# jurgisp/pydreamer

Measured on AMD Instinct MI355X. Metric: grad-steps/sec (world-model+AC) at B=50,T=50,H=15, 64×64 obs, 1/2/4/8 GPU, higher is better.
Workload: dtype f32; 1 GPU; atari-literal: defaults+atari, batch_size 50, batch_length 50, imag_horizon 15, deter_dim 600, stoch 32x32, hidden 1000, cnn_depth 48, action_dim 18, fp32; fwd + 4 bwd + clip + 4 AdamW per step; replay resident in HBM; global_batch=50, batch_length=50, imag_horizon=15, parallelism=dp1 (batch-sharded [50])

## Files before the change

### include/dreamer_hip.h

```cpp
#ifndef DREAMER_HIP_H
#define DREAMER_HIP_H

#include <stddef.h>
#include <stdint.h>

#ifdef __cplusplus
extern "C" {
#endif

#define DM_OK 0
#define DM_E_SHAPE (-1)
#define DM_E_WORKSPACE (-2)
#define DM_E_HIP (-3)
#define DM_E_DEVICE (-4)
#define DM_E_NULL (-5)

#define DM_MAX_MLP_LAYERS 8

typedef struct dm_shape {
  int32_t T, B, I;
  int32_t H;
  int32_t D, Hd;
  int32_t S, C;
  int32_t E;
  int32_t A;
  int32_t mlp_hidden;
  int32_t mlp_layers;
  int32_t cnn_depth;
  int32_t img, img_ch;
  int32_t flags;
} dm_shape;
#define DM_FLAG_IMAGE_U8 16
#define DM_FLAG_GRU_SHIFT 5
#define DM_FLAG_BF16 128
#define DM_FLAG_GRU_LAYERS_SHIFT 8
#define DM_FLAG_GRU_LAYERS_MASK (3 << DM_FLAG_GRU_LAYERS_SHIFT)
#define DM_FLAG_GRU_MASK (3 << DM_FLAG_GRU_SHIFT)

int dm_version(void);
const char* dm_last_error(void);
int dm_device_check(void);
size_t dm_workspace_bytes(const dm_shape* shp);
int dm_stream_create_cu_mask(const uint32_t* mask, int words, void** stream);
int dm_stream_destroy(void* stream);
int dm_wgrad_side_arm(int on);
int dm_wgrad_side_touch(void);
int dm_wgrad_side_join(void* stream);

#define DM_GEMM_ACCUM 1
#define DM_GEMM_ELU 2
#define DM_GEMM_BF16 256
int dm_gemm_f32(int a_layout, int b_layout, int M, int N, int K,
                const float* A, int lda, const float* B, int ldb, float* C, int ldc,
                const float* bias, const float* add, int ldadd, int flags,
                void* ws, size_t ws_bytes, void* stream);
int dm_gemm_bf16h(int a_layout, int b_layout, int M, int N, int K, const uint16_t* A, int lda, const uint16_t* B, int ldb,
                  float* C, int ldc, uint16_t* C_h, const float* bias, int flags, void* ws, size_t ws_bytes, void* stream);
int dm_bf16_twins_enable(int on);
int dm_gemm_dma_enable(int on);
int dm_convt_kskip_enable(int on);
int dm_kl_staged_enable(int on);
int dm_dec_l4_bwd_direct_enable(int on);
int dm_dec_l4_fwd_shared_enable(int on);
int dm_rssm_lds_enable(int on);
int dm_bptt_fold_enable(int on);
int dm_rssm_lds_status(void);
int dm_rssm_lds_status_ack(void);
int dm_rssm_lds_gave_up(void);
int dm_rssm_lds_prof(unsigned long long* out16, int reset);

int dm_ln_elu_fwd(int rows, int n, const float* x, int ldx, const float* gamma, const float* beta, float eps,
                  float* y, int ldy, float* stats, void* stream);
int dm_ln_elu_bwd(int rows, int n, const float* x, int ldx, const float* y, int ldy, const float* stats,
                  const float* gamma, const float* dy, int lddy, float* dx, int lddx,
                  float* dgamma, float* dbeta, void* ws, size_t ws_bytes, void* stream);
int dm_colsum(int rows, int n, const float* x, int ld, float* out, void* ws, size_t ws_bytes, void* stream);

int dm_gru_gates_fwd(int rows, int D, const float* gi, const float* gh, const float* h_in, int ldh,
                     float* h_out, int ldo, void* stream);
int dm_gru_gates_bwd(int rows, int D, const float* gi, const float* gh, const float* h_in, int ldh,
                     const float* dh_out, int lddh, float* dgi, float* dgh, float* dh_in, int lddi, void* stream);

int dm_sample_onehot(int rows, int groups, int C, const float* logits, int ldl, const float* u,
                     const int32_t* forced_idx, float* onehot, int ldo, int32_t* idx, void* stream);

int dm_kl_balance_fwd(int rows, int S, int C, const float* post, const float* prior,
                      float* kl, float* ent_post, float* ent_prior, void* stream);
int dm_kl_balance_bwd(int rows, int S, int C, const float* post, const float* prior,
                      float scale_post, float scale_prior, float* dpost, float* dprior, void* stream);
int dm_st_softmax_bwd(int rows, int groups, int C, const float* logits, int ldl, const float* dz, int lddz,
                      float* dlogits, int lddl, int accum, void* stream);

int dm_kl_sampled_fwd(int rows, int S, int C, const float* post, const float* prior, const int32_t* idx, float* out, void* stream);
int dm_kl_sampled_bwd(int rows, int S, int C, const float* post, const float* prior, const int32_t* idx, float scale,
                      const float* row_w, float* dpost, float* dprior, void* stream);
int dm_kl_sampled_gauss_fwd(int rows, int S, const float* post, const float* prior, const float* z, int ldz, float* out,
                            void* stream);
int dm_kl_sampled_gauss_bwd(int rows, int S, const float* post, const float* prior, const float* z, int ldz, float scale,
                            const float* row_w, float* dpost, float* dprior, float* dz, int lddz, void* stream);
int dm_reduce_i(int TB, int I, int W, const float* x, int mode, float* out, float* w_out, void* stream);
int dm_combine_rows(int count, int64_t n, const float* const* x, const float* w, float* out, void* stream);
int dm_scale_rows(int64_t rows, int n, float* x, int ldx, const float* w, float scale, void* stream);

int dm_mask_rows(int rows, int n, const float* x, int ldx, const uint8_t* reset, float* y, int ldy, void* stream);

int dm_im2col_s2(int n, int hb, int wb, int c, int k, const float* big, int big_nchw, float* col, void* stream);
#define DM_C2I_ELU 1
int dm_col2im_s2(int n, int hb, int wb, int c, int k, const float* col, const float* bias, int flags,
                 const float* elu_ref, float* big, void* stream);

typedef struct dm_mlp_params {
  const float* w[DM_MAX_MLP_LAYERS + 1];
  const float* b[DM_MAX_MLP_LAYERS + 1];
  const float* ln_g[DM_MAX_MLP_LAYERS];
  const float* ln_b[DM_MAX_MLP_LAYERS];
  int32_t precision;
  int32_t reserved_;
} dm_mlp_params;
typedef struct dm_mlp_grads {
  float* w[DM_MAX_MLP_LAYERS + 1];
  float* b[DM_MAX_MLP_LAYERS + 1];
  float* ln_g[DM_MAX_MLP_LAYERS];
  float* ln_b[DM_MAX_MLP_LAYERS];
} dm_mlp_grads;
size_t dm_mlp_acts_floats(int rows, int hidden, int layers);
size_t dm_mlp_ws_floats(int rows, int hidden, int layers);
int dm_mlp_head_fwd(int rows, int in_dim, int hidden, int layers, int out_dim,
                    const float* x, int ldx, const dm_mlp_params* p, float* acts, float* out,
                    void* ws, size_t ws_bytes, void* stream);
int dm_mlp_head_fwd_sparse(int rows, int in_dim, int sparse_cols, int hidden, int layers, int out_dim,
                           const float* x, int ldx, const dm_mlp_params* p, float* acts, float* out,
                           void* ws, size_t ws_bytes, void* stream);
int dm_mlp_head_fwd_rows(int rows_total, int row0, int rows, int in_dim, int sparse_cols, int hidden, int layers, int out_dim,
                         const float* x, int ldx, const dm_mlp_params* p, float* acts, float* out,
                         void* ws, size_t ws_bytes, void* stream);

int dm_mlp_head_bwd(int rows, int in_dim, int hidden, int layers, int out_dim,
                    const float* x, int ldx, const dm_mlp_params* p, const float* acts, const float* dout,
                    const dm_mlp_grads* g, float* dx, int lddx, int dx_accum,
                    void* ws, size_t ws_bytes, void* stream);

int dm_head_loss(int kind, int rows, const float* out, const float* target, float scale, float loss_const,
                 float* loss, float* dout, float* mean_out, void* stream);

int dm_head_loss_normal_nd(int rows, int V, const float* out, const float* target, float scale, float loss_const,
                           float* loss, float* dout, float* mean_out, void* stream);
// ... 163 lines not shown
```

### pydreamer_amd/csrc/conv_direct.hip

```cpp
#include "common.h"

static inline int grid_for_px(size_t total, int per_block) { return (int)((total + per_block - 1) / per_block); }


template <int CO, bool U8, bool FB = false>
__global__ void __launch_bounds__(256) enc_l1_fwd_kernel(int npix, const void* __restrict__ image_,
                                                         const float* __restrict__ wt, const float* __restrict__ bias,
                                                         float* __restrict__ y, unsigned short* __restrict__ y_h) {
  const int p = blockIdx.x * 256 + threadIdx.x;
  const bool ok = p < npix;
  const int pc = ok ? p : npix - 1;
  const int n = pc / 961, r = pc - n * 961, py = r / 31, px = r - py * 31;
  float acc[CO];
  if (FB) {
    const float4* fb = reinterpret_cast<const float4*>(bias + (size_t)n * CO);
#pragma unroll
    for (int o = 0; o < CO; o += 4) {
      const float4 b4 = fb[o >> 2];
      acc[o] = b4.x; acc[o + 1] = b4.y; acc[o + 2] = b4.z; acc[o + 3] = b4.w;
    }
  } else {
#pragma unroll
    for (int o = 0; o < CO; ++o) acc[o] = bias[o];
  }
#pragma unroll 1
  for (int cy = 0; cy < 12; ++cy) {
    const int c = cy >> 2, ky = cy & 3;
    float v[4];
    if (U8) {
      const uint8_t* img = (const uint8_t*)image_ + (size_t)n * 12288 + ((size_t)(2 * py + ky) * 64 + 2 * px) * 3 + c;
#pragma unroll
      for (int kx = 0; kx < 4; ++kx) v[kx] = (float)img[kx * 3] / 255.0f - 0.5f;
    } else {
      const float* img = (const float*)image_ + (size_t)n * 12288 + (size_t)c * 4096 + (2 * py + ky) * 64 + 2 * px;
      const float2 a = *reinterpret_cast<const float2*>(img), b = *reinterpret_cast<const float2*>(img + 2);
      v[0] = a.x; v[1] = a.y; v[2] = b.x; v[3] = b.y;
    }
    const float* w = wt + (size_t)(c * 16 + ky * 4) * CO;
#pragma unroll
    for (int kx = 0; kx < 4; ++kx)
#pragma unroll
      for (int o = 0; o < CO; ++o) acc[o] = fmaf(v[kx], w[kx * CO + o], acc[o]);
  }
  if (ok) {
    float4* dst = reinterpret_cast<float4*>(y + (size_t)p * CO);
#pragma unroll
    for (int o = 0; o < CO; o += 4)
      dst[o >> 2] = make_float4(dm_elu(acc[o]), dm_elu(acc[o + 1]), dm_elu(acc[o + 2]), dm_elu(acc[o + 3]));
    if (y_h) {
      uint2* dh = reinterpret_cast<uint2*>(y_h + (size_t)p * CO);
#pragma unroll
      for (int o = 0; o < CO; o += 4)
        dh[o >> 2] = dm_pack_bf16x4(make_float4(dm_elu(acc[o]), dm_elu(acc[o + 1]), dm_elu(acc[o + 2]), dm_elu(acc[o + 3])));
    }
  }
}

template <int WROW = 48>
__global__ void __launch_bounds__(256) enc_l1_wt_kernel(int co, const float* __restrict__ w, float* __restrict__ wt) {
  const int e = blockIdx.x * 256 + threadIdx.x;
  if (e < co * 48) wt[e] = w[(size_t)(e % co) * WROW + e / co];
}
__global__ void __launch_bounds__(256) enc_l1_fb_kernel(int frames, int co, const float* __restrict__ w5,
                                                        const float* __restrict__ bias, const float* __restrict__ reward,
                                                        const float* __restrict__ terminal, float* __restrict__ fb) {
  const int e = blockIdx.x * 256 + threadIdx.x;
  if (e >= frames * co) return;
  const int n = e / co, o = e - n * co;
  const float* w = w5 + (size_t)o * 80 + 48;
  float s3 = 0.f, s4 = 0.f;
#pragma unroll
  for (int t = 0; t < 16; ++t) { s3 += w[t]; s4 += w[16 + t]; }
  fb[e] = fmaf(terminal[n], s4, fmaf(reward[n], s3, bias[o]));
}

bool dm_enc_l1_direct_ok(int ch, int d, int img) {
  return ch == 3 && img == 64 && (d == 8 || d == 16 || d == 32 || d == 48 || d == 64);
}
int dm_enc_l1_fwd_launch(int frames, int d, int u8, const void* image, const float* w, const float* bias, float* wt,
                         float* y, unsigned short* y_h, hipStream_t st) {
  if (frames <= 0) return DM_OK;
  hipLaunchKernelGGL(enc_l1_wt_kernel<48>, dim3(grid_for_px((size_t)d * 48, 256)), dim3(256), 0, st, d, w, wt);
  DM_LAUNCH_CHECK();
  const int npix = frames * 961;
  const dim3 grid(grid_for_px((size_t)npix, 256)), blk(256);
#define DM_ENC_L1(CO_)                                                                                              \
  if (d == CO_) {                                                                                                   \
    if (u8) hipLaunchKernelGGL((enc_l1_fwd_kernel<CO_, true>), grid, blk, 0, st, npix, image, wt, bias, y, y_h);      \
    else hipLaunchKernelGGL((enc_l1_fwd_kernel<CO_, false>), grid, blk, 0, st, npix, image, wt, bias, y, y_h);        \
  }
  DM_ENC_L1(8) DM_ENC_L1(16) DM_ENC_L1(32) DM_ENC_L1(48) DM_ENC_L1(64)
#undef DM_ENC_L1
  DM_LAUNCH_CHECK();
  return DM_OK;
}

int dm_enc_l1_fwd_planes_launch(int frames, int d, int u8, const void* image, const float* w5, const float* bias,
                                const float* reward, const float* terminal, float* wt, float* fb, float* y,
                                unsigned short* y_h, hipStream_t st) {
  if (frames <= 0) return DM_OK;
  hipLaunchKernelGGL(enc_l1_wt_kernel<80>, dim3(grid_for_px((size_t)d * 48, 256)), dim3(256), 0, st, d, w5, wt);
  DM_LAUNCH_CHECK();
  hipLaunchKernelGGL(enc_l1_fb_kernel, dim3(grid_for_px((size_t)frames * d, 256)), dim3(256), 0, st, frames, d, w5, bias, reward,
                     terminal, fb);
  DM_LAUNCH_CHECK();
  const int npix = frames * 961;
  const dim3 grid(grid_for_px((size_t)npix, 256)), blk(256);
#define DM_ENC_L1P(CO_)                                                                                             \
  if (d == CO_) {                                                                                                   \
    if (u8) hipLaunchKernelGGL((enc_l1_fwd_kernel<CO_, true, true>), grid, blk, 0, st, npix, image, wt, fb, y, y_h);  \
    else hipLaunchKernelGGL((enc_l1_fwd_kernel<CO_, false, true>), grid, blk, 0, st, npix, image, wt, fb, y, y_h);    \
  }
  DM_ENC_L1P(8) DM_ENC_L1P(16) DM_ENC_L1P(32) DM_ENC_L1P(48) DM_ENC_L1P(64)
#undef DM_ENC_L1P
  DM_LAUNCH_CHECK();
  return DM_OK;
}

typedef float f32x4c __attribute__((ext_vector_type(4)));
constexpr int ENC_LD = 68;
template <int OB, bool U8>
__global__ void __launch_bounds__(256) enc_l1_wgrad_kernel(int frames, int CO, const void* __restrict__ image_,
                                                           const float* __restrict__ G, float* __restrict__ part) {
  __shared__ __attribute__((aligned(16))) float img[3 * 64 * ENC_LD];
  const int tid = threadIdx.x, lane = tid & 63, wave = tid >> 6;
  const int l15 = lane & 15, q = lane >> 4;
  f32x4c acc[OB][3];
#pragma unroll
  for (int i = 0; i < OB; ++i)
#pragma unroll
    for (int j = 0; j < 3; ++j) acc[i][j] = (f32x4c){0.f, 0.f, 0.f, 0.f};
  const int tapoff = (l15 >> 2) * ENC_LD + (l15 & 3);
  for (int n = blockIdx.x; n < frames; n += gridDim.x) {
    __syncthreads();
    if (U8) {
      const uint8_t* src = (const uint8_t*)image_ + (size_t)n * 12288;
      for (int e = tid; e < 12288; e += 256) {
        const int c = e % 3, pix = e / 3;
        img[(c * 64 + (pix >> 6)) * ENC_LD + (pix & 63)] = (float)src[e] / 255.0f - 0.5f;
      }
    } else {
      const float4* src = reinterpret_cast<const float4*>((const float*)image_ + (size_t)n * 12288);
      for (int e = tid; e < 3072; e += 256) {
        const int row = e >> 4, c4 = e & 15;
        *reinterpret_cast<float4*>(&img[row * ENC_LD + 4 * c4]) = src[e];
      }
    }
    __syncthreads();
    const float* Gn = G + (size_t)n * 961 * CO;
    for (int p0 = wave * 64; p0 < 961; p0 += 256) {
      float a[16][OB];
#pragma unroll
      for (int ks = 0; ks < 16; ++ks) {
        const int p = p0 + 4 * ks + q;
        const int pc = p < 961 ? p : 960;
#pragma unroll
        for (int ob = 0; ob < OB; ++ob) {
          const int o = ob * 16 + l15;
          a[ks][ob] = Gn[(size_t)pc * CO + (o < CO ? o : CO - 1)] * ((p < 961 && o < CO) ? 1.f : 0.f);
        }
      }
#pragma unroll
      for (int ks = 0; ks < 16; ++ks) {
        const int p = p0 + 4 * ks + q;
        const int pc = p < 961 ? p : 960;
        const int py = pc / 31, px = pc - py * 31;
        const float* base = &img[2 * py * ENC_LD + 2 * px + tapoff];
        float b[3];
#pragma unroll
        for (int c = 0; c < 3; ++c) b[c] = base[c * 64 * ENC_LD];
#pragma unroll
        for (int ob = 0; ob < OB; ++ob)
#pragma unroll
          for (int c = 0; c < 3; ++c) acc[ob][c] = __builtin_amdgcn_mfma_f32_16x16x4f32(a[ks][ob], b[c], acc[ob][c], 0, 0, 0);
      }
    }
  }
  float* dst = part + (size_t)(blockIdx.x * 4 + wave) * CO * 48;
#pragma unroll
  for (int ob = 0; ob < OB; ++ob)
#pragma unroll
    for (int c = 0; c < 3; ++c)
#pragma unroll
      for (int r = 0; r < 4; ++r) {
        const int o = ob * 16 + 4 * q + r;
        if (o < CO) dst[(size_t)o * 48 + c * 16 + l15] = acc[ob][c][r];
      }
}

static int enc_l1_wgrad_blocks(int frames) { return frames > 512 ? 512 : frames; }
size_t dm_enc_l1_wgrad_part_floats(int frames, int d) { return (size_t)enc_l1_wgrad_blocks(frames) * 4 * d * 48; }
int dm_enc_l1_wgrad_launch(int frames, int d, int u8, const void* image, const float* G, float* part, float* dW, void* ws,
                           size_t ws_bytes, hipStream_t st) {
  if (frames <= 0) return DM_OK;
  const int blocks = enc_l1_wgrad_blocks(frames);
  const dim3 grid(blocks), blk(256);
  const int OB = (d + 15) / 16;
  DM_REQUIRE(OB >= 1 && OB <= 4, DM_E_SHAPE, "enc_l1_wgrad: cnn_depth %d", d);
#define DM_ENC_WG(OB_)                                                                                               \
  if (OB == OB_) {                                                                                                   \
    if (u8) hipLaunchKernelGGL((enc_l1_wgrad_kernel<OB_, true>), grid, blk, 0, st, frames, d, image, G, part);         \
    else hipLaunchKernelGGL((enc_l1_wgrad_kernel<OB_, false>), grid, blk, 0, st, frames, d, image, G, part);           \
  }
  DM_ENC_WG(1) DM_ENC_WG(2) DM_ENC_WG(3) DM_ENC_WG(4)
#undef DM_ENC_WG
  DM_LAUNCH_CHECK();
  return dm_colsum_launch(blocks * 4, d * 48, part, d * 48, dW, ws, ws_bytes, st);
}

__global__ void __launch_bounds__(256) enc_l1_planes_colsum_kernel(int frames, int d, int W, int frames_per_chunk,
                                                                   const float* __restrict__ G, const float* __restrict__ reward,
                                                                   const float* __restrict__ terminal, float* __restrict__ part) {
  __shared__ float sh[3][256];
  const int tid = threadIdx.x;
  const int n0 = blockIdx.x * frames_per_chunk, n1 = min(frames, n0 + frames_per_chunk);
  const int fl = 961 * d;
  float a0 = 0.f, a1 = 0.f, a2 = 0.f;
  if (tid < W)
    for (int n = n0; n < n1; ++n) {
      const float* x = G + (size_t)n * fl;
      float b0 = 0.f, b1 = 0.f, b2 = 0.f, b3 = 0.f;
      int i = tid;
      for (; i + 3 * W < fl; i += 4 * W) {
        b0 += x[i];
        b1 += x[i + W];
        b2 += x[i + 2 * W];
        b3 += x[i + 3 * W];
      }
      for (; i < fl; i += W) b0 += x[i];
      const float s = (b0 + b1) + (b2 + b3);
      a0 += s;
      a1 = fmaf(reward[n], s, a1);
      a2 = fmaf(terminal[n], s, a2);
    }
  sh[0][tid] = a0; sh[1][tid] = a1; sh[2][tid] = a2;
  __syncthreads();
  if (tid < 3 * d) {
    const int q = tid / d, o = tid - q * d;
    float s = 0.f;
    for (int t = o; t < W; t += d) s += sh[q][t];
    part[((size_t)blockIdx.x * 3 + q) * d + o] = s;
  }
}
__global__ void __launch_bounds__(256) enc_l1_planes_final_kernel(int d, int chunks, const float* __restrict__ part,
                                                                  const float* __restrict__ dw3, float* __restrict__ db,
                                                                  float* __restrict__ dW5) {
  __shared__ float sums[3 * 64];
  const int tid = threadIdx.x;
  if (tid < 3 * d) {
    const float* p = part + tid;
    const size_t st = (size_t)3 * d;
    float s = 0.f;
    int c = 0;
    for (; c + 3 < chunks; c += 4) {
      const float v0 = p[(size_t)c * st], v1 = p[(size_t)(c + 1) * st], v2 = p[(size_t)(c + 2) * st], v3 = p[(size_t)(c + 3) * st];
      s += v0; s += v1; s += v2; s += v3;
    }
    for (; c < chunks; ++c) s += p[(size_t)c * st];
// ... 445 lines not shown
```

### pydreamer_amd/hip.py

```python
import ctypes
import os
from ctypes import POINTER, Structure, c_char_p, c_float, c_int, c_int32, c_int64, c_size_t, c_void_p

import torch

_HERE = os.path.dirname(os.path.abspath(__file__))
LIB_PATH = os.environ.get('DM_LIB_PATH') or os.path.join(_HERE, 'libdreamer_hip.so')

DM_MAX_MLP_LAYERS = 8
DM_GEMM_ACCUM = 1
DM_GEMM_ELU = 2
DM_C2I_ELU = 1
DM_FLAG_IMAGE_U8 = 16
DM_FLAG_BF16 = 128
DM_GEMM_BF16 = 256

RSSM_PARAM_ORDER = [
    'z_mlp.weight', 'z_mlp.bias', 'a_mlp.weight', 'in_norm.weight', 'in_norm.bias',
    'gru.layers.0.weight_ih', 'gru.layers.0.weight_hh', 'gru.layers.0.bias_ih', 'gru.layers.0.bias_hh',
    'prior_mlp_h.weight', 'prior_mlp_h.bias', 'prior_norm.weight', 'prior_norm.bias', 'prior_mlp.weight', 'prior_mlp.bias',
    'post_mlp_h.weight', 'post_mlp_h.bias', 'post_mlp_e.weight', 'post_norm.weight', 'post_norm.bias',
    'post_mlp.weight', 'post_mlp.bias',
]
GRU_KINDS = {'gru': 0, 'gru_layernorm': 1, 'gru_layernorm_dv2': 2}
# ... 104 lines not shown
    'dm_ln_elu_bwd': (c_int, [c_int, c_int, _P, c_int, _P, c_int, _P, _P, _P, c_int, _P, c_int, _P, _P, _P, c_size_t, _P]),
    'dm_colsum': (c_int, [c_int, c_int, _P, c_int, _P, _P, c_size_t, _P]),
    'dm_gru_gates_fwd': (c_int, [c_int, c_int, _P, _P, _P, c_int, _P, c_int, _P]),
    'dm_gru_gates_bwd': (c_int, [c_int, c_int, _P, _P, _P, c_int, _P, c_int, _P, _P, _P, c_int, _P]),
    'dm_sample_onehot': (c_int, [c_int, c_int, c_int, _P, c_int, _P, _P, _P, c_int, _P, _P]),
    'dm_kl_balance_fwd': (c_int, [c_int, c_int, c_int, _P, _P, _P, _P, _P, _P]),
    'dm_kl_balance_bwd': (c_int, [c_int, c_int, c_int, _P, _P, c_float, c_float, _P, _P, _P]),
    'dm_st_softmax_bwd': (c_int, [c_int, c_int, c_int, _P, c_int, _P, c_int, _P, c_int, c_int, _P]),
    'dm_mask_rows': (c_int, [c_int, c_int, _P, c_int, _P, _P, c_int, _P]),
    'dm_kl_sampled_fwd': (c_int, [c_int, c_int, c_int, _P, _P, _P, _P, _P]),
    'dm_kl_sampled_bwd': (c_int, [c_int, c_int, c_int, _P, _P, _P, c_float, _P, _P, _P, _P]),
    'dm_kl_sampled_gauss_fwd': (c_int, [c_int, c_int, _P, _P, _P, c_int, _P, _P]),
    'dm_kl_sampled_gauss_bwd': (c_int, [c_int, c_int, _P, _P, _P, c_int, c_float, _P, _P, _P, _P, c_int, _P]),
    'dm_reduce_i': (c_int, [c_int, c_int, c_int, _P, c_int, _P, _P, _P]),
    'dm_combine_rows': (c_int, [c_int, c_int64, POINTER(c_void_p), POINTER(c_float), _P, _P]),
    'dm_scale_rows': (c_int, [c_int64, c_int, _P, c_int, _P, c_float, _P]),
    'dm_im2col_s2': (c_int, [c_int, c_int, c_int, c_int, c_int, _P, c_int, _P, _P]),
    'dm_col2im_s2': (c_int, [c_int, c_int, c_int, c_int, c_int, _P, _P, c_int, _P, _P, _P]),
    'dm_mlp_acts_floats': (c_size_t, [c_int, c_int, c_int]),
    'dm_mlp_ws_floats': (c_size_t, [c_int, c_int, c_int]),
    'dm_mlp_head_fwd': (c_int, [c_int, c_int, c_int, c_int, c_int, _P, c_int, POINTER(dm_mlp_params), _P, _P, _P,
                                c_size_t, _P]),
    'dm_mlp_head_fwd_sparse': (c_int, [c_int, c_int, c_int, c_int, c_int, c_int, _P, c_int, POINTER(dm_mlp_params), _P, _P, _P, c_size_t, _P]),
    'dm_mlp_head_bwd': (c_int, [c_int, c_int, c_int, c_int, c_int, _P, c_int, POINTER(dm_mlp_params), _P, _P,
                                POINTER(dm_mlp_grads), _P, c_int, c_int, _P, c_size_t, _P]),
    'dm_head_loss': (c_int, [c_int, c_int, _P, _P, c_float, c_float, _P, _P, _P, _P]),
    'dm_head_loss_normal_nd': (c_int, [c_int, c_int, _P, _P, c_float, c_float, _P, _P, _P, _P]),
    'dm_cat_target_index': (c_int, [c_int, c_int, c_int, _P, _P, _P]),
    'dm_cat_image_loss': (c_int, [c_int, c_int, c_int, c_int, _P, c_int, _P, _P, _P, _P]),
    'dm_cat_image_pred': (c_int, [c_int, c_int, c_int, c_int, _P, c_int, _P, _P, _P, _P, _P, _P]),
    'dm_cat_concat_rows': (c_int, [c_int, c_int, c_int, c_int, _P, c_int, _P, _P, _P]),
    'dm_dense_image_rows': (c_int, [c_int, c_int, c_int, _P, _P, _P, _P, _P, c_int, _P]),
    'dm_elu_rows_fwd': (c_int, [c_int, c_int, _P, c_int, _P, c_int, _P]),
    'dm_elu_rows_bwd': (c_int, [c_int, c_int, _P, c_int, _P, c_int, _P, c_int, _P]),
    'dm_cat_image_loss_mix': (c_int, [c_int, c_int, c_int, c_int, _P, c_int, _P, c_float, _P, _P, _P]),
    'dm_goals_stats_ws_floats': (c_size_t, [c_int, c_int]),
    'dm_goals_stats': (c_int, [c_int, c_int, _P, _P, _P, _P, _P, c_size_t, _P]),
    'dm_preprocess_image_u8': (c_int, [c_int64, c_int, c_int, _P, _P, _P]),
    'dm_conv_encoder_acts_floats': (c_size_t, [POINTER(dm_shape)]),
    'dm_conv_encoder_fwd': (c_int, [POINTER(dm_shape), _P, POINTER(dm_conv_params), _P, _P, _P, c_size_t, _P]),
    'dm_conv_encoder_bwd': (c_int, [POINTER(dm_shape), _P, POINTER(dm_conv_params), _P, _P, POINTER(dm_conv_grads), _P,
                                    c_size_t, _P]),
    'dm_conv_encoder_fwd_planes': (c_int, [POINTER(dm_shape), _P, POINTER(dm_conv_params), _P, _P, _P, _P, c_int, _P, c_size_t, _P]),
    'dm_conv_encoder_bwd_planes': (c_int, [POINTER(dm_shape), _P, POINTER(dm_conv_params), _P, _P, _P, _P, c_int,
                                           POINTER(dm_conv_grads), _P, c_size_t, _P]),
    'dm_conv_decoder_acts_floats': (c_size_t, [POINTER(dm_shape)]),
    'dm_conv_decoder_pred_offset': (c_size_t, [POINTER(dm_shape)]),
    'dm_conv_decoder_mse_fwd': (c_int, [POINTER(dm_shape), _P, c_int, _P, POINTER(dm_conv_params), _P, _P, _P, _P,
                                        c_size_t, _P]),
    'dm_conv_decoder_mse_bwd': (c_int, [POINTER(dm_shape), _P, c_int, _P, POINTER(dm_conv_params), _P, c_float,
                                        POINTER(dm_conv_grads), _P, c_int, _P, c_size_t, _P]),
    'dm_conv_decoder_mse_bwd_rows': (c_int, [POINTER(dm_shape), _P, c_int, _P, POINTER(dm_conv_params), _P, c_float, _P,
                                             POINTER(dm_conv_grads), _P, c_int, _P, c_size_t, _P]),
    'dm_rssm_acts_floats': (c_size_t, [POINTER(dm_shape)]),
    'dm_rssm_sequence_fwd': (c_int, [POINTER(dm_shape), _P, _P, _P, _P, _P, _P, _P, POINTER(dm_rssm_params), _P, _P, _P,
                                     _P, _P, _P, c_size_t, _P]),
    'dm_rssm_sequence_bwd': (c_int, [POINTER(dm_shape), _P, _P, _P, POINTER(dm_rssm_params), _P, _P, _P, _P, _P, _P,
                                     POINTER(dm_rssm_grads), _P, _P, c_size_t, _P]),
    'dm_dream_rollout': (c_int, [POINTER(dm_shape), c_int, _P, POINTER(dm_rssm_params), POINTER(dm_mlp_params), _P, _P,
                                 _P, _P, _P, _P, _P, _P, c_size_t, _P]),
    'dm_gae_losses': (c_int, [c_int, c_int, c_float, c_float, _P, _P, _P, _P, _P, _P, _P, _P]),
    'dm_actor_loss': (c_int, [c_int, c_int, _P, _P, _P, _P, c_float, c_float, _P, _P, _P, _P]),
    'dm_critic_loss': (c_int, [c_int, _P, _P, _P, c_float, _P, _P, _P]),
    'dm_sample_continuous': (c_int, [c_int, c_int, c_int, _P, _P, _P, _P]),
    'dm_actor_loss_continuous': (c_int, [c_int, c_int, c_int, _P, _P, _P, _P, c_float, c_float, _P, _P, _P, _P]),
    'dm_multi_sum': (c_int, [c_int, POINTER(dm_reduce_item), _P, _P]),
    'dm_combine': (c_int, [c_int, _P, POINTER(c_float), _P, _P]),
    'dm_multi_tensor_norm_clip': (c_int, [_P, c_int64, c_float, _P, _P, c_size_t, _P]),
    'dm_scale_inplace': (c_int, [_P, c_int64, _P, _P]),
    'dm_adamw_step': (c_int, [_P, _P, _P, _P, c_int64, c_float, c_float, c_float, c_float, c_float, c_int, _P, _P]),
    'dm_copy_params': (c_int, [_P, _P, c_int64, _P]),
    'dm_axpby': (c_int, [c_int64, c_float, _P, c_float, _P, _P]),
    'dm_prof_begin': (c_int, [c_int]),
    'dm_prof_end': (c_int, [POINTER(ctypes.c_double), c_int]),
    'dm_prof_rows': (c_int, [POINTER(ctypes.c_double), c_int]),
    'dm_mlp_chain_min_rows': (c_int, [c_int]),
    'dm_rollout_fuse_act_enable': (c_int, [c_int]),
    'dm_bf16_twins_enable': (c_int, [c_int]),
    'dm_gemm_dma_enable': (c_int, [c_int]),
    'dm_convt_kskip_enable': (c_int, [c_int]),
    'dm_kl_staged_enable': (c_int, [c_int]),
    'dm_dec_l4_bwd_direct_enable': (c_int, [c_int]),
    'dm_dec_l4_fwd_shared_enable': (c_int, [c_int]),
    'dm_rssm_lds_enable': (c_int, [c_int]),
    'dm_bptt_fold_enable': (c_int, [c_int]),
    'dm_rssm_lds_status': (c_int, []),
    'dm_rssm_lds_status_ack': (c_int, []),
    'dm_rssm_lds_gave_up': (c_int, []),
    'dm_rssm_lds_prof': (c_int, [_P, c_int]),
    'dm_rssm_last_schedule': (c_int, [c_int]),
    'dm_wgrad_side_arm': (c_int, [c_int]),
    'dm_wgrad_side_touch': (c_int, []),
    'dm_wgrad_side_join': (c_int, [_P]),
    'dm_dream_rollout_marks': (c_int, [c_int, POINTER(c_int), POINTER(c_void_p)]),
    'dm_mlp_head_fwd_rows': (c_int, [c_int, c_int, c_int, c_int, c_int, c_int, c_int, c_int, _P, c_int, POINTER(dm_mlp_params), _P, _P, _P,
                                     c_size_t, _P]),
    'dm_replay_gather': (c_int, [c_int, c_int, c_int, POINTER(dm_replay_field), _P, _P, _P]),
    'dm_gru_sequence_acts_floats': (c_size_t, [c_int, c_int, c_int, c_int]),
    'dm_gru_sequence_ws_bytes': (c_size_t, [c_int, c_int, c_int, c_int]),
    'dm_gru_sequence_fwd': (c_int, [c_int, c_int, c_int, c_int, _P, c_int, _P, _P, POINTER(dm_gru_params), _P, _P, c_int,
                                    _P, c_size_t, _P]),
    'dm_gru_sequence_bwd': (c_int, [c_int, c_int, c_int, c_int, _P, c_int, POINTER(dm_gru_params), _P, _P, c_int, _P, c_int,
                                    POINTER(dm_gru_grads), _P, c_int, _P, c_size_t, _P]),
    'dm_gru_sequence_last_schedule': (c_int, []),
    'dm_gru_sequence_fuse_enable': (c_int, [c_int]),
    'dm_policy_draw_ws_floats': (c_size_t, [c_int]),
    'dm_policy_draw': (c_int, [c_int, c_int, c_int, _P, c_int, _P, _P, _P, c_int, _P, _P, _P, _P, _P, c_size_t, _P]),
    'dm_policy_draw_mode': (c_int, [c_int, c_int, c_float, c_int, c_int, _P, c_int, _P, _P, _P, _P, c_int, _P, _P, _P, _P, _P, c_size_t,
                                    _P]),
}

_lib = None
DM_ABI_VERSION = 16


def lib():
    global _lib
    if _lib is None:
        if not os.path.exists(LIB_PATH):
            raise DreamerHipError(
                f'{LIB_PATH} not found: build it with `python -c "import __graft_entry__ as g; g.build()"` '
                f'(or `make -C pydreamer_amd/csrc`). There is no CPU fallback for the training path.')
        handle = ctypes.CDLL(LIB_PATH)
        for name, (restype, argtypes) in _SIGNATURES.items():
            fn = getattr(handle, name)
            fn.restype = restype
            fn.argtypes = argtypes
        if handle.dm_version() != DM_ABI_VERSION:
            raise DreamerHipError(f'{LIB_PATH} has ABI version {handle.dm_version()}, this binding is written for '
                                  f'{DM_ABI_VERSION}: rebuild it (`make -C pydreamer_amd/csrc`)')
        _lib = handle
    return _lib


def exported_symbols():
    return sorted(_SIGNATURES)


def call(name, *args):
    fn = getattr(lib(), name)
    rc = fn(*args)
    if rc != 0:
        msg = lib().dm_last_error().decode('utf-8', 'replace')
        raise DreamerHipError(f'{name} failed with code {rc}: {msg}')
    return rc


def last_schedule(which):
    word = int(lib().dm_rssm_last_schedule(which))
    if word < 0:
        raise DreamerHipError(f'dm_rssm_last_schedule({which}): no such entry point')
    bits = (SCHED_FWD, SCHED_BWD, SCHED_ROLL)[which]
    out = {k: bool(word & v) for k, v in bits.items()}
    if which == 1:
        out['nchunk'] = (word >> SCHED_BWD_NCHUNK_SHIFT) & 15
    return out


def ptr(t):
    if t is None:
        return None
    if not t.is_cuda:
        raise DreamerHipError(f'expected a CUDA/HIP tensor, got device {t.device} (no CPU path)')
    if not t.is_contiguous():
        raise DreamerHipError(f'expected a contiguous tensor, got strides {t.stride()} for shape {tuple(t.shape)}')
    return c_void_p(t.data_ptr())
# ... 64 lines not shown
```

Measured before the change: 30.80 grad-steps/s.

## Use MFMA for encoder layer-1 forward conv and software-pipeline its wgrad loads

Adds an MFMA-based forward kernel for the first encoder conv, enabled by default. It stages each frame's image in LDS, keeps the weights in registers, and prefetches the next frame while the current one computes. This replaces the per-pixel scalar FMA kernel and its separate weight-transpose launch. The layer-1 weight-gradient kernel also double-buffers its gradient loads in chunks of 8 so the next chunk is fetched while MFMAs run on the current one. The costs are higher register pressure and more complex boundary handling; only the forward path can be switched off by a flag.

After: 30.90 grad-steps/s, median of 6. About the same (+0.3%).

```diff
diff --git a/include/dreamer_hip.h b/include/dreamer_hip.h
--- a/include/dreamer_hip.h
+++ b/include/dreamer_hip.h
@@ -62,6 +62,7 @@
 int dm_kl_staged_enable(int on);
 int dm_dec_l4_bwd_direct_enable(int on);
 int dm_dec_l4_fwd_shared_enable(int on);
+int dm_enc_l1_fwd_mfma_enable(int on);
 int dm_rssm_lds_enable(int on);
 int dm_bptt_fold_enable(int on);
 int dm_rssm_lds_status(void);
diff --git a/pydreamer_amd/csrc/conv_direct.hip b/pydreamer_amd/csrc/conv_direct.hip
--- a/pydreamer_amd/csrc/conv_direct.hip
+++ b/pydreamer_amd/csrc/conv_direct.hip
@@ -74,12 +74,139 @@
   fb[e] = fmaf(terminal[n], s4, fmaf(reward[n], s3, bias[o]));
 }
 
+typedef float f32x4c __attribute__((ext_vector_type(4)));
+constexpr int ENC_LD = 68;
+constexpr int ENCM_WGS = 768;
+template <int CB, bool U8, bool FB>
+__global__ void __launch_bounds__(256) enc_l1_fwd_mfma_kernel(int frames, int d, const void* __restrict__ image_,
+                                                              const float* __restrict__ w, const float* __restrict__ bias,
+                                                              float* __restrict__ y, unsigned short* __restrict__ y_h) {
+  constexpr int WROW = FB ? 80 : 48;
+  constexpr int NPRE = U8 ? 3 : 12;
+  __shared__ __attribute__((aligned(16))) float img[3 * 64 * ENC_LD];
+  const int tid = threadIdx.x, lane = tid & 63, wave = tid >> 6;
+  const int l15 = lane & 15, q = lane >> 4;
+  float wreg[12][CB];
+#pragma unroll
+  for (int cb = 0; cb < CB; ++cb) {
+    const int o = 16 * cb + l15;
+    const float* wo = w + (size_t)(o < d ? o : d - 1) * WROW + q;
+#pragma unroll
+    for (int s = 0; s < 12; ++s) {
+      const float v = wo[4 * s];
+      wreg[s][cb] = o < d ? v : 0.f;
+    }
+  }
+  int c0c[CB];
+  f32x4c cin[CB], cnext[CB];
+#pragma unroll
+  for (int cb = 0; cb < CB; ++cb) {
+    c0c[cb] = 16 * cb + 4 * q < d ? 16 * cb + 4 * q : 0;
+    if (!FB) cin[cb] = (f32x4c){bias[c0c[cb]], bias[c0c[cb] + 1], bias[c0c[cb] + 2], bias[c0c[cb] + 3]};
+  }
+  f32x4c pre[NPRE];
+  auto fetch = [&](int n) {
+    const f32x4c* src = reinterpret_cast<const f32x4c*>(U8 ? (const char*)image_ + (size_t)n * 12288
+                                                          : (const char*)image_ + (size_t)n * 12288 * sizeof(float));
+#pragma unroll
+    for (int i = 0; i < NPRE; ++i) pre[i] = src[tid + 256 * i];
+    if (FB) {
+#pragma unroll
+      for (int cb = 0; cb < CB; ++cb) {
+        const float4 f = *reinterpret_cast<const float4*>(bias + (size_t)n * d + c0c[cb]);
+        cnext[cb] = (f32x4c){f.x, f.y, f.z, f.w};
+      }
+    }
+  };
+  const int px = 16 * (wave & 1) + l15;
+  const int pxc = px < 31 ? px : 30;
+  int n = blockIdx.x;
+  if (n < frames) fetch(n);
+  for (; n < frames; n += gridDim.x) {
+    __syncthreads();
+#pragma unroll
+    for (int i = 0; i < NPRE; ++i) {
+      const int e = tid + 256 * i;
+      if (U8) {
+#pragma unroll
+        for (int j = 0; j < 16; ++j) {
+          const int b = 16 * e + j, c = b % 3, pix = b / 3;
+          const unsigned byte = (__float_as_uint(pre[i][j >> 2]) >> (8 * (j & 3))) & 255u;
+          img[(c * 64 + (pix >> 6)) * ENC_LD + (pix & 63)] = (float)byte / 255.0f - 0.5f;
+        }
+      } else {
+        *reinterpret_cast<f32x4c*>(&img[(e >> 4) * ENC_LD + 4 * (e & 15)]) = pre[i];
+      }
+    }
+    if (FB) {
+#pragma unroll
+      for (int cb = 0; cb < CB; ++cb) cin[cb] = cnext[cb];
+    }
+    __syncthreads();
+    if (n + (int)gridDim.x < frames) fetch(n + gridDim.x);
+    const float* col = &img[2 * pxc + q];
+    float b[12], bn[12];
+    auto patch = [&](int py, float (&dst)[12]) {
+#pragma unroll
+      for (int s = 0; s < 12; ++s) dst[s] = col[((s >> 2) * 64 + 2 * py + (s & 3)) * ENC_LD];
+    };
+    patch(wave >> 1, b);
+    for (int py = wave >> 1; py < 31; py += 2) {
+      patch(py + 2 < 31 ? py + 2 : 30, bn);
+      f32x4c acc[CB];
+#pragma unroll
+      for (int cb = 0; cb < CB; ++cb) acc[cb] = cin[cb];
+#pragma unroll
+      for (int s = 0; s < 12; ++s)
+#pragma unroll
+        for (int cb = 0; cb < CB; ++cb) acc[cb] = __builtin_amdgcn_mfma_f32_16x16x4f32(wreg[s][cb], b[s], acc[cb], 0, 0, 0);
+      if (px < 31) {
+        const size_t row = ((size_t)n * 961 + py * 31 + px) * d;
+#pragma unroll
+        for (int cb = 0; cb < CB; ++cb) {
+          const int c0 = 16 * cb + 4 * q;
+          if (c0 < d) {
+            const float4 v = make_float4(dm_elu(acc[cb][0]), dm_elu(acc[cb][1]), dm_elu(acc[cb][2]), dm_elu(acc[cb][3]));
+            *reinterpret_cast<float4*>(y + row + c0) = v;
+            if (y_h) *reinterpret_cast<uint2*>(y_h + row + c0) = dm_pack_bf16x4(v);
+          }
+        }
+      }
+#pragma unroll
+      for (int s = 0; s < 12; ++s) b[s] = bn[s];
+    }
+  }
+}
+
+static int g_enc_l1_mfma = 1;
+extern "C" int dm_enc_l1_fwd_mfma_enable(int on) {
+  if (on >= 0) g_enc_l1_mfma = on ? 1 : 0;
+  return g_enc_l1_mfma;
+}
+
 bool dm_enc_l1_direct_ok(int ch, int d, int img) {
   return ch == 3 && img == 64 && (d == 8 || d == 16 || d == 32 || d == 48 || d == 64);
+}
+template <bool FB>
+static int enc_l1_fwd_mfma_launch(int frames, int d, int u8, const void* image, const float* w, const float* c, float* y,
+                                  unsigned short* y_h, hipStream_t st) {
+  DM_REQUIRE(dm_enc_l1_direct_ok(3, d, 64), DM_E_SHAPE, "enc_l1_fwd: cnn_depth %d", d);
+  const dim3 grid(frames < ENCM_WGS ? frames : ENCM_WGS), blk(256);
+  const int CB = (d + 15) / 16;
+#define DM_ENC_L1M(CB_)                                                                                               \
+  if (CB == CB_) {                                                                                                    \
+    if (u8) hipLaunchKernelGGL((enc_l1_fwd_mfma_kernel<CB_, true, FB>), grid, blk, 0, st, frames, d, image, w, c, y, y_h);   \
+    else hipLaunchKernelGGL((enc_l1_fwd_mfma_kernel<CB_, false, FB>), grid, blk, 0, st, frames, d, image, w, c, y, y_h);     \
+  }
+  DM_ENC_L1M(1) DM_ENC_L1M(2) DM_ENC_L1M(3) DM_ENC_L1M(4)
+#undef DM_ENC_L1M
+  DM_LAUNCH_CHECK();
+  return DM_OK;
 }
 int dm_enc_l1_fwd_launch(int frames, int d, int u8, const void* image, const float* w, const float* bias, float* wt,
                          float* y, unsigned short* y_h, hipStream_t st) {
   if (frames <= 0) return DM_OK;
+  if (g_enc_l1_mfma) return enc_l1_fwd_mfma_launch<false>(frames, d, u8, image, w, bias, y, y_h, st);
   hipLaunchKernelGGL(enc_l1_wt_kernel<48>, dim3(grid_for_px((size_t)d * 48, 256)), dim3(256), 0, st, d, w, wt);
   DM_LAUNCH_CHECK();
   const int npix = frames * 961;
@@ -99,10 +226,11 @@
                                 const float* reward, const float* terminal, float* wt, float* fb, float* y,
                                 unsigned short* y_h, hipStream_t st) {
   if (frames <= 0) return DM_OK;
-  hipLaunchKernelGGL(enc_l1_wt_kernel<80>, dim3(grid_for_px((size_t)d * 48, 256)), dim3(256), 0, st, d, w5, wt);
-  DM_LAUNCH_CHECK();
   hipLaunchKernelGGL(enc_l1_fb_kernel, dim3(grid_for_px((size_t)frames * d, 256)), dim3(256), 0, st, frames, d, w5, bias, reward,
                      terminal, fb);
+  DM_LAUNCH_CHECK();
+  if (g_enc_l1_mfma) return enc_l1_fwd_mfma_launch<true>(frames, d, u8, image, w5, fb, y, y_h, st);
+  hipLaunchKernelGGL(enc_l1_wt_kernel<80>, dim3(grid_for_px((size_t)d * 48, 256)), dim3(256), 0, st, d, w5, wt);
   DM_LAUNCH_CHECK();
   const int npix = frames * 961;
   const dim3 grid(grid_for_px((size_t)npix, 256)), blk(256);
@@ -117,8 +245,6 @@
   return DM_OK;
 }
 
-typedef float f32x4c __attribute__((ext_vector_type(4)));
-constexpr int ENC_LD = 68;
 template <int OB, bool U8>
 __global__ void __launch_bounds__(256) enc_l1_wgrad_kernel(int frames, int CO, const void* __restrict__ image_,
                                                            const float* __restrict__ G, float* __restrict__ part) {
@@ -131,7 +257,41 @@
 #pragma unroll
     for (int j = 0; j < 3; ++j) acc[i][j] = (f32x4c){0.f, 0.f, 0.f, 0.f};
   const int tapoff = (l15 >> 2) * ENC_LD + (l15 & 3);
+  constexpr int NK = 8;
+  const std::integral_constant<int, NK> k8{};
+  const std::integral_constant<int, 1> k1{};
+  auto load = [&](const float* Gn, int p0, float (&dst)[NK][OB], auto nks) {
+#pragma unroll
+    for (int ks = 0; ks < decltype(nks)::value; ++ks) {
+      const int p = p0 + 4 * ks + q;
+      const int pc = p < 961 ? p : 960;
+#pragma unroll
+      for (int ob = 0; ob < OB; ++ob) {
+        const int o = ob * 16 + l15;
+        dst[ks][ob] = Gn[(size_t)pc * CO + (o < CO ? o : CO - 1)] * ((p < 961 && o < CO) ? 1.f : 0.f);
+      }
+    }
+  };
+  auto mma = [&](int p0, const float (&a)[NK][OB], auto nks) {
+#pragma unroll
+    for (int ks = 0; ks < decltype(nks)::value; ++ks) {
+      const int p = p0 + 4 * ks + q;
+      const int pc = p < 961 ? p : 960;
+      const int py = pc / 31, px = pc - py * 31;
+      const float* base = &img[2 * py * ENC_LD + 2 * px + tapoff];
+      float b[3];
+#pragma unroll
+      for (int c = 0; c < 3; ++c) b[c] = base[c * 64 * ENC_LD];
+#pragma unroll
+      for (int ob = 0; ob < OB; ++ob)
+#pragma unroll
+        for (int c = 0; c < 3; ++c) acc[ob][c] = __builtin_amdgcn_mfma_f32_16x16x4f32(a[ks][ob], b[c], acc[ob][c], 0, 0, 0);
+    }
+  };
   for (int n = blockIdx.x; n < frames; n += gridDim.x) {
+    const float* Gn = G + (size_t)n * 961 * CO;
+    float a[NK][OB], an[NK][OB];
+    load(Gn, wave * 64, a, k8);
     __syncthreads();
     if (U8) {
       const uint8_t* src = (const uint8_t*)image_ + (size_t)n * 12288;
@@ -147,33 +307,18 @@
       }
     }
     __syncthreads();
-    const float* Gn = G + (size_t)n * 961 * CO;
-    for (int p0 = wave * 64; p0 < 961; p0 += 256) {
-      float a[16][OB];
-#pragma unroll
-      for (int ks = 0; ks < 16; ++ks) {
-        const int p = p0 + 4 * ks + q;
-        const int pc = p < 961 ? p : 960;
-#pragma unroll
-        for (int ob = 0; ob < OB; ++ob) {
-          const int o = ob * 16 + l15;
-          a[ks][ob] = Gn[(size_t)pc * CO + (o < CO ? o : CO - 1)] * ((p < 961 && o < CO) ? 1.f : 0.f);
-        }
-      }
-#pragma unroll
-      for (int ks = 0; ks < 16; ++ks) {
-        const int p = p0 + 4 * ks + q;
-        const int pc = p < 961 ? p : 960;
-        const int py = pc / 31, px = pc - py * 31;
-        const float* base = &img[2 * py * ENC_LD + 2 * px + tapoff];
-        float b[3];
-#pragma unroll
-        for (int c = 0; c < 3; ++c) b[c] = base[c * 64 * ENC_LD];
-#pragma unroll
-        for (int ob = 0; ob < OB; ++ob)
-#pragma unroll
-          for (int c = 0; c < 3; ++c) acc[ob][c] = __builtin_amdgcn_mfma_f32_16x16x4f32(a[ks][ob], b[c], acc[ob][c], 0, 0, 0);
-      }
+#pragma unroll 1
+    for (int p0 = wave * 64; p0 < 961;) {
+      const int pn = (p0 & 32) ? p0 + 224 : p0 + 32;
+      if (pn + 32 <= 961) load(Gn, pn, an, k8);
+      else if (pn < 961) load(Gn, pn, an, k1);
+      if (p0 + 32 <= 961) mma(p0, a, k8);
+      else mma(p0, a, k1);
+#pragma unroll
+      for (int ks = 0; ks < NK; ++ks)
+#pragma unroll
+        for (int ob = 0; ob < OB; ++ob) a[ks][ob] = an[ks][ob];
+      p0 = pn;
     }
   }
   float* dst = part + (size_t)(blockIdx.x * 4 + wave) * CO * 48;
diff --git a/pydreamer_amd/hip.py b/pydreamer_amd/hip.py
--- a/pydreamer_amd/hip.py
+++ b/pydreamer_amd/hip.py
@@ -210,6 +210,7 @@
     'dm_kl_staged_enable': (c_int, [c_int]),
     'dm_dec_l4_bwd_direct_enable': (c_int, [c_int]),
     'dm_dec_l4_fwd_shared_enable': (c_int, [c_int]),
+    'dm_enc_l1_fwd_mfma_enable': (c_int, [c_int]),
     'dm_rssm_lds_enable': (c_int, [c_int]),
     'dm_bptt_fold_enable': (c_int, [c_int]),
     'dm_rssm_lds_status': (c_int, []),
```

## Add MFMA-based encoder first-layer conv forward kernel with LDS-staged frames

Applied to the files above, without the earlier changes.

Adds a new forward kernel for the first encoder convolution. Each workgroup stages a whole 64x64x3 frame in shared memory and prefetches the next frame into registers, then computes 16-pixel blocks with 16x16x4 f32 MFMA instructions against weights held in registers. It replaces the per-pixel scalar FMA kernel, which re-read the image from global memory for every output pixel. It is enabled by default when the image pointer is 16-byte aligned and uses a persistent grid capped at 512 workgroups, which may leave some units idle or change occupancy.

Result: no change. 30.93 grad-steps/s before, 30.94 grad-steps/s after (median of 2 runs) (+0.0%).

```diff
diff --git a/include/dreamer_hip.h b/include/dreamer_hip.h
--- a/include/dreamer_hip.h
+++ b/include/dreamer_hip.h
@@ -62,6 +62,7 @@
 int dm_kl_staged_enable(int on);
 int dm_dec_l4_bwd_direct_enable(int on);
 int dm_dec_l4_fwd_shared_enable(int on);
+int dm_enc_l1_fwd_mfma_enable(int on);
 int dm_rssm_lds_enable(int on);
 int dm_bptt_fold_enable(int on);
 int dm_rssm_lds_status(void);
diff --git a/pydreamer_amd/csrc/conv_direct.hip b/pydreamer_amd/csrc/conv_direct.hip
--- a/pydreamer_amd/csrc/conv_direct.hip
+++ b/pydreamer_amd/csrc/conv_direct.hip
@@ -74,23 +74,131 @@
   fb[e] = fmaf(terminal[n], s4, fmaf(reward[n], s3, bias[o]));
 }
 
+typedef float f32x4c __attribute__((ext_vector_type(4)));
+constexpr int ENC_LD = 68;
+constexpr int ENCM_WGS = 512, ENCM_BLOCKS = 61;
+template <int CO, bool U8, bool FB>
+__global__ void __launch_bounds__(256) enc_l1_fwd_mfma_kernel(int frames, const void* __restrict__ image_,
+                                                              const float* __restrict__ wt, const float* __restrict__ bias,
+                                                              float* __restrict__ y, unsigned short* __restrict__ y_h) {
+  constexpr int OB = (CO + 15) / 16;
+  constexpr int NPRE = U8 ? 3 : 12;
+  __shared__ __attribute__((aligned(16))) float img[3 * 64 * ENC_LD];
+  const int tid = threadIdx.x, lane = tid & 63, wave = tid >> 6;
+  const int l15 = lane & 15, q = lane >> 4;
+  float wa[12][OB];
+#pragma unroll
+  for (int cy = 0; cy < 12; ++cy)
+#pragma unroll
+    for (int ob = 0; ob < OB; ++ob) {
+      const int o = ob * 16 + l15;
+      wa[cy][ob] = o < CO ? wt[(size_t)(cy * 4 + q) * CO + o] : 0.f;
+    }
+  f32x4c c0[OB];
+#pragma unroll
+  for (int ob = 0; ob < OB; ++ob) {
+    c0[ob] = (f32x4c){0.f, 0.f, 0.f, 0.f};
+    if (!FB && ob * 16 + 4 * q < CO) {
+#pragma unroll
+      for (int r = 0; r < 4; ++r) c0[ob][r] = bias[ob * 16 + 4 * q + r];
+    }
+  }
+  typedef unsigned u32x4 __attribute__((ext_vector_type(4)));
+  u32x4 pre[NPRE];
+  const u32x4* frame = reinterpret_cast<const u32x4*>(image_) + tid;
+  int n = blockIdx.x;
+  if (n < frames) {
+#pragma unroll
+    for (int i = 0; i < NPRE; ++i) pre[i] = frame[(size_t)n * (NPRE * 256) + 256 * i];
+  }
+  for (; n < frames; n += gridDim.x) {
+    __syncthreads();
+#pragma unroll
+    for (int i = 0; i < NPRE; ++i) {
+      const int e = tid + 256 * i;
+      if (U8) {
+#pragma unroll
+        for (int j = 0; j < 16; ++j) {
+          const int b = 16 * e + j, pix = b / 3, c = b - 3 * pix;
+          img[(c * 64 + (pix >> 6)) * ENC_LD + (pix & 63)] = (float)((pre[i][j >> 2] >> (8 * (j & 3))) & 255u) / 255.0f - 0.5f;
+        }
+      } else {
+        const int row = e >> 4, c4 = e & 15;
+        *reinterpret_cast<u32x4*>(&img[row * ENC_LD + 4 * c4]) = pre[i];
+      }
+    }
+    __syncthreads();
+    if (n + (int)gridDim.x < frames) {
+#pragma unroll
+      for (int i = 0; i < NPRE; ++i) pre[i] = frame[(size_t)(n + gridDim.x) * (NPRE * 256) + 256 * i];
+    }
+    if (FB) {
+#pragma unroll
+      for (int ob = 0; ob < OB; ++ob)
+        if (ob * 16 + 4 * q < CO) c0[ob] = *reinterpret_cast<const f32x4c*>(bias + (size_t)n * CO + ob * 16 + 4 * q);
+    }
+    for (int blk = (wave + n) & 3; blk < ENCM_BLOCKS; blk += 4) {
+      const int p = blk * 16 + l15;
+      const int pc = p < 961 ? p : 960;
+      const int py = pc / 31, px = pc - py * 31;
+      const float* src = &img[2 * py * ENC_LD + 2 * px + q];
+      f32x4c acc[OB];
+#pragma unroll
+      for (int ob = 0; ob < OB; ++ob) acc[ob] = c0[ob];
+#pragma unroll
+      for (int cy = 0; cy < 12; ++cy) {
+        const float b = src[((cy >> 2) * 64 + (cy & 3)) * ENC_LD];
+#pragma unroll
+        for (int ob = 0; ob < OB; ++ob) acc[ob] = __builtin_amdgcn_mfma_f32_16x16x4f32(wa[cy][ob], b, acc[ob], 0, 0, 0);
+      }
+      if (p < 961) {
+        const size_t off = ((size_t)n * 961 + p) * CO + 4 * q;
+#pragma unroll
+        for (int ob = 0; ob < OB; ++ob) {
+          if (ob * 16 + 4 * q >= CO) continue;
+          const float4 v = make_float4(dm_elu(acc[ob][0]), dm_elu(acc[ob][1]), dm_elu(acc[ob][2]), dm_elu(acc[ob][3]));
+          *reinterpret_cast<float4*>(y + off + ob * 16) = v;
+          if (y_h) *reinterpret_cast<uint2*>(y_h + off + ob * 16) = dm_pack_bf16x4(v);
+        }
+      }
+    }
+  }
+}
+
+static int g_enc_l1_fwd_mfma = 1;
+extern "C" int dm_enc_l1_fwd_mfma_enable(int on) {
+  if (on >= 0) g_enc_l1_fwd_mfma = on ? 1 : 0;
+  return g_enc_l1_fwd_mfma;
+}
+
 bool dm_enc_l1_direct_ok(int ch, int d, int img) {
   return ch == 3 && img == 64 && (d == 8 || d == 16 || d == 32 || d == 48 || d == 64);
+}
+template <bool FB>
+static void enc_l1_fwd_kernels(int frames, int d, int u8, const void* image, const float* wt, const float* b, float* y,
+                               unsigned short* y_h, hipStream_t st) {
+  const bool mfma = g_enc_l1_fwd_mfma && ((uintptr_t)image & 15) == 0;
+  const int npix = frames * 961;
+  const dim3 grid(mfma ? (frames < ENCM_WGS ? frames : ENCM_WGS) : grid_for_px((size_t)npix, 256)), blk(256);
+#define DM_ENC_L1(CO_)                                                                                              \
+  if (d == CO_) {                                                                                                   \
+    if (mfma) {                                                                                                     \
+      if (u8) hipLaunchKernelGGL((enc_l1_fwd_mfma_kernel<CO_, true, FB>), grid, blk, 0, st, frames, image, wt, b, y, y_h);   \
+      else hipLaunchKernelGGL((enc_l1_fwd_mfma_kernel<CO_, false, FB>), grid, blk, 0, st, frames, image, wt, b, y, y_h);     \
+    } else {                                                                                                        \
+      if (u8) hipLaunchKernelGGL((enc_l1_fwd_kernel<CO_, true, FB>), grid, blk, 0, st, npix, image, wt, b, y, y_h);   \
+      else hipLaunchKernelGGL((enc_l1_fwd_kernel<CO_, false, FB>), grid, blk, 0, st, npix, image, wt, b, y, y_h);     \
+    }                                                                                                               \
+  }
+  DM_ENC_L1(8) DM_ENC_L1(16) DM_ENC_L1(32) DM_ENC_L1(48) DM_ENC_L1(64)
+#undef DM_ENC_L1
 }
 int dm_enc_l1_fwd_launch(int frames, int d, int u8, const void* image, const float* w, const float* bias, float* wt,
                          float* y, unsigned short* y_h, hipStream_t st) {
   if (frames <= 0) return DM_OK;
   hipLaunchKernelGGL(enc_l1_wt_kernel<48>, dim3(grid_for_px((size_t)d * 48, 256)), dim3(256), 0, st, d, w, wt);
   DM_LAUNCH_CHECK();
-  const int npix = frames * 961;
-  const dim3 grid(grid_for_px((size_t)npix, 256)), blk(256);
-#define DM_ENC_L1(CO_)                                                                                              \
-  if (d == CO_) {                                                                                                   \
-    if (u8) hipLaunchKernelGGL((enc_l1_fwd_kernel<CO_, true>), grid, blk, 0, st, npix, image, wt, bias, y, y_h);      \
-    else hipLaunchKernelGGL((enc_l1_fwd_kernel<CO_, false>), grid, blk, 0, st, npix, image, wt, bias, y, y_h);        \
-  }
-  DM_ENC_L1(8) DM_ENC_L1(16) DM_ENC_L1(32) DM_ENC_L1(48) DM_ENC_L1(64)
-#undef DM_ENC_L1
+  enc_l1_fwd_kernels<false>(frames, d, u8, image, wt, bias, y, y_h, st);
   DM_LAUNCH_CHECK();
   return DM_OK;
 }
@@ -104,21 +212,11 @@
   hipLaunchKernelGGL(enc_l1_fb_kernel, dim3(grid_for_px((size_t)frames * d, 256)), dim3(256), 0, st, frames, d, w5, bias, reward,
                      terminal, fb);
   DM_LAUNCH_CHECK();
-  const int npix = frames * 961;
-  const dim3 grid(grid_for_px((size_t)npix, 256)), blk(256);
-#define DM_ENC_L1P(CO_)                                                                                             \
-  if (d == CO_) {                                                                                                   \
-    if (u8) hipLaunchKernelGGL((enc_l1_fwd_kernel<CO_, true, true>), grid, blk, 0, st, npix, image, wt, fb, y, y_h);  \
-    else hipLaunchKernelGGL((enc_l1_fwd_kernel<CO_, false, true>), grid, blk, 0, st, npix, image, wt, fb, y, y_h);    \
-  }
-  DM_ENC_L1P(8) DM_ENC_L1P(16) DM_ENC_L1P(32) DM_ENC_L1P(48) DM_ENC_L1P(64)
-#undef DM_ENC_L1P
+  enc_l1_fwd_kernels<true>(frames, d, u8, image, wt, fb, y, y_h, st);
   DM_LAUNCH_CHECK();
   return DM_OK;
 }
 
-typedef float f32x4c __attribute__((ext_vector_type(4)));
-constexpr int ENC_LD = 68;
 template <int OB, bool U8>
 __global__ void __launch_bounds__(256) enc_l1_wgrad_kernel(int frames, int CO, const void* __restrict__ image_,
                                                            const float* __restrict__ G, float* __restrict__ part) {
diff --git a/pydreamer_amd/hip.py b/pydreamer_amd/hip.py
--- a/pydreamer_amd/hip.py
+++ b/pydreamer_amd/hip.py
@@ -210,6 +210,7 @@
     'dm_kl_staged_enable': (c_int, [c_int]),
     'dm_dec_l4_bwd_direct_enable': (c_int, [c_int]),
     'dm_dec_l4_fwd_shared_enable': (c_int, [c_int]),
+    'dm_enc_l1_fwd_mfma_enable': (c_int, [c_int]),
     'dm_rssm_lds_enable': (c_int, [c_int]),
     'dm_bptt_fold_enable': (c_int, [c_int]),
     'dm_rssm_lds_status': (c_int, []),
```
